# facebookresearch/habitat-lab

Hardware: NVIDIA H100
Metric: DD-PPO learner frames/sec (ResNet18 RGB-D 256x256) (higher is better)
Workload: dtype bf16

## Files before the change

habitat-lab_b200/csrc/conv.cu:

```cuda
#include "common.cuh"
#include "wgmma.cuh"

namespace hb200 {
void count_launch(int n);
static int g_umma_layout = 1;

using namespace wg;

constexpr int kStages = 3;
constexpr int kTileM = 128;
constexpr int kMaxBN = 128;
constexpr int kChunkK = 64;
constexpr int kMaxChunks = 512;

template <int LAYOUT>
__device__ __forceinline__ uint32_t tile_off(int row, int k8, int rows_total) {
  if (LAYOUT == 0) return (uint32_t)(k8 * rows_total + row) << 4;
  return (uint32_t)((row >> 3) << 10) + (uint32_t)((row & 7) << 7) + (uint32_t)((k8 ^ (row & 7)) << 4);
}
template <int LAYOUT>
__device__ __forceinline__ uint64_t kmajor_desc(uint32_t base, int kk, int rows_total) {
  if (LAYOUT == 0)
    return make_smem_desc(base + (uint32_t)(kk * 2 * rows_total * 16), (uint32_t)rows_total * 16, 128, kNoSwizzle);
  return make_smem_desc(base + (uint32_t)(kk * 32), 16, 1024, kSwizzle128B);
}
template <int LAYOUT>
constexpr uint32_t kmajor_hi() { return LAYOUT == 0 ? 8 * 128 : 8 * 1024; }

struct ConvArgs {
  const __nv_bfloat16* src;
  const __nv_bfloat16* wimg;
  __nv_bfloat16* out;
  const __nv_bfloat16* addend;
  double* stats;
  int B, SH, SW, SC;
  int OH, OW, OC;
  int kh, kw, stride, pad;
  int M, nchunks, cshift, gn_groups;
  const float* bias;
  int relu;
  int s2_classes;
  int wbn;
};

template <int BN, int MODE, int LAYOUT, int NST = kStages>
__global__ void __launch_bounds__(128) conv_igemm_kernel(const ConvArgs a) {
  extern __shared__ __align__(16) uint8_t smem_raw[];
  __shared__ float stage_buf[kStageFloats];
  constexpr uint32_t kABytes = kTileM * kChunkK * 2;
  constexpr uint32_t kBBytes = BN * kChunkK * 2;
  constexpr uint32_t kStageBytes = kABytes + kBBytes;
  static_assert(BN <= kMaxBN, "conv: N tile");
  const uint32_t smem_base = (smem_u32(smem_raw) + 1023u) & ~1023u;

  const int tid = threadIdx.x, lane = tid & 31;
  const int n0 = blockIdx.y * BN;
  __shared__ short chunk_ids[kMaxChunks];
  __shared__ int n_valid_s;
  int m, ob, op, oq, ph = 0, pw = 0;
  bool row_ok;
  if (MODE == 1 && a.s2_classes) {
    const int mq = a.M >> 2;
    const int tiles_per_class = (mq + kTileM - 1) / kTileM;
    const int cls = blockIdx.x / tiles_per_class;
    const int idx = (blockIdx.x - cls * tiles_per_class) * kTileM + tid;
    ph = cls >> 1; pw = cls & 1;
    row_ok = idx < mq;
    const int h2 = a.OH >> 1, w2 = a.OW >> 1;
    const int ii = row_ok ? idx : 0;
    ob = ii / (h2 * w2);
    const int rem = ii - ob * (h2 * w2);
    op = 2 * (rem / w2) + ph;
    oq = 2 * (rem % w2) + pw;
    m = (ob * a.OH + op) * a.OW + oq;
  } else {
    m = blockIdx.x * kTileM + tid;
    row_ok = m < a.M;
    const int hw = a.OH * a.OW;
    const int mm = row_ok ? m : 0;
    ob = mm / hw;
    const int rem = mm - ob * hw;
    op = rem / a.OW;
    oq = rem - op * a.OW;
  }
  __shared__ int4 row_info[kTileM];
  if (LAYOUT == 1) row_info[tid] = make_int4(ob, op, oq, row_ok ? 1 : 0);
  if (tid == 0) {
    int nv = 0;
    const int cpt = a.SC >> 6;
    for (int c = 0; c < a.nchunks && nv < kMaxChunks; ++c) {
      bool ok = true;
      if (MODE == 1 && a.s2_classes) {
        const int tap = c / cpt;
        const int r = tap / a.kw, sx = tap - r * a.kw;
        ok = tap < a.kh * a.kw && (((ph + a.pad - r) & 1) == 0) && (((pw + a.pad - sx) & 1) == 0);
      }
      if (ok) chunk_ids[nv++] = (short)c;
    }
    n_valid_s = nv;
  }

  __syncthreads();
  const int n_valid = n_valid_s;
  const int taps = a.kh * a.kw;
  const int wbn = a.wbn;
  const __nv_bfloat16* wtile =
// ... 748 lines not shown
```

habitat-lab_b200/csrc/conv_halo.cu:

```cuda
#include <cuda.h>
#include <stdlib.h>

#include "common.cuh"
#include "wgmma.cuh"

namespace hb200 {
void count_launch(int n);
using namespace wg;

constexpr int TH = 16, TW = 8;

__device__ __forceinline__ float warp_reduce16(float (&v)[16], int lane) {
  float a[8], b[4], c[2];
  const bool b4 = lane & 16, b3 = lane & 8, b2 = lane & 4, b1 = lane & 2;
#pragma unroll
  for (int i = 0; i < 8; ++i) a[i] = (b4 ? v[i + 8] : v[i]) + __shfl_xor_sync(0xffffffffu, b4 ? v[i] : v[i + 8], 16);
#pragma unroll
  for (int i = 0; i < 4; ++i) b[i] = (b3 ? a[i + 4] : a[i]) + __shfl_xor_sync(0xffffffffu, b3 ? a[i] : a[i + 4], 8);
#pragma unroll
  for (int i = 0; i < 2; ++i) c[i] = (b2 ? b[i + 2] : b[i]) + __shfl_xor_sync(0xffffffffu, b2 ? b[i] : b[i + 2], 4);
  float d = (b1 ? c[1] : c[0]) + __shfl_xor_sync(0xffffffffu, b1 ? c[0] : c[1], 2);
  d += __shfl_xor_sync(0xffffffffu, d, 1);
  return d;
}
// ... 806 lines not shown
            const uint64_t db = make_smem_desc(s_w + (r * KW + s) * (C * N * 2) + 2 * kk * (N * 16), N * 16, 128, kNoSwizzle);
            mma128<N, kT>(acc_t, da, 8 * ATOM, db, accum);
            accum = 1;
          }
      wgmma_commit();
      wgmma_wait<0>();
      acc_fence(acc_t);
    }
    if (NB == 1 && tid == 0 && it + 1 < my_n) issue_halo(first + (it + 1) * stride, 0);
    {
      int b, oh0, ow0;
      tile_coords(first + it * stride, b, oh0, ow0);
      const size_t pix = ((size_t)b * a.H + oh0 + py) * a.W + ow0 + px;
#pragma unroll
      for (int col0 = 0; col0 < N; col0 += 32) {
        float acc[32];
        acc_row32(acc_t, col0, stage_buf, acc);
        if (MODE == 0 && a.stats != nullptr)
          halo_gn_stats_chunk(acc, lane, N / a.gn_groups, a.stats + (size_t)b * a.gn_groups * 2, col0);
        const size_t o = pix * N + col0;
        if (MODE == 1 && a.addend != nullptr) {
          const uint4* ad = reinterpret_cast<const uint4*>(a.addend + o);
#pragma unroll
          for (int v = 0; v < 4; ++v) {
            float f[8];
            unpack8(ad[v], f);
#pragma unroll
            for (int e = 0; e < 8; ++e) acc[v * 8 + e] += f[e];
          }
        }
        uint4* dst = reinterpret_cast<uint4*>(a.y + o);
#pragma unroll
        for (int v = 0; v < 4; ++v) {
          uint4 u;
          if (MODE == 0) {
            u.x = pack_f16x2(acc[v * 8 + 0], acc[v * 8 + 1]);
            u.y = pack_f16x2(acc[v * 8 + 2], acc[v * 8 + 3]);
            u.z = pack_f16x2(acc[v * 8 + 4], acc[v * 8 + 5]);
            u.w = pack_f16x2(acc[v * 8 + 6], acc[v * 8 + 7]);
          } else {
            u.x = pack_bf16x2(acc[v * 8 + 0], acc[v * 8 + 1]);
            u.y = pack_bf16x2(acc[v * 8 + 2], acc[v * 8 + 3]);
            u.z = pack_bf16x2(acc[v * 8 + 4], acc[v * 8 + 5]);
            u.w = pack_bf16x2(acc[v * 8 + 6], acc[v * 8 + 7]);
          }
          dst[v] = u;
        }
      }
    }
  }
}


template <int C, int N, int KH, int KW, int PAD, int MODE, int NS, bool SW = false>
__global__ void __launch_bounds__(160)
conv_halo_ws_kernel(const HaloArgs a, const __grid_constant__ CUtensorMap tmap) {
  using Cfg = HaloCfg<C, N, KH, KW, PAD>;
  constexpr int CJ = Cfg::CJ, HH = Cfg::HH, HWD = Cfg::HWD;
  constexpr uint32_t SLAB = (uint32_t)((HH * HWD * 16 + 127) / 128 * 128);
  constexpr uint32_t RB = C * 2, ATOM = 8 * RB, COPY = HH * ATOM;
  constexpr uint32_t STAGE = SW ? KW * COPY : CJ * SLAB;
  constexpr int kSw = RB == 128 ? kSwizzle128B : kSwizzle64B;
  static_assert(!SW || RB == 64 || RB == 128, "swizzled halo copies: 32 or 64 channels");
  extern __shared__ __align__(16) uint8_t smem_raw[];
  __shared__ __align__(8) uint64_t full_bar[NS], empty_bar[NS];
  __shared__ float stage_buf[kStageFloats];
  const uint32_t sbase = (smem_u32(smem_raw) + 1023u) & ~1023u;
  const uint32_t s_w = sbase;
  const uint32_t s_halo0 = s_w + Cfg::W_BYTES;
  const int tid = threadIdx.x, warp = tid >> 5, lane = tid & 31;
  if (tid == 0) {
#pragma unroll
    for (int i = 0; i < NS; ++i) { mbar_init(&full_bar[i], 1); mbar_init(&empty_bar[i], 1); }
    mbar_fence_init();
  }
  {
    const uint4* src = reinterpret_cast<const uint4*>(a.wimg);
    for (int v = tid; v < Cfg::W_BYTES / 16; v += blockDim.x) cp_async16(s_w + (uint32_t)v * 16, src + v, true);
  }
  cp_async_commit();
  cp_async_wait<0>();
  fence_proxy_async_smem();
  __syncthreads();
  const int tiles_x = a.W / TW, tiles_per_img = tiles_x * (a.H / TH);
  const int first = blockIdx.x, stride = gridDim.x;
  const int my_n = first < a.ntiles ? (a.ntiles - first + stride - 1) / stride : 0;
  const CUtensorMap* const tmap_p = &tmap;

  if (warp == 4) {
    if (lane == 0) {
      for (int it = 0; it < my_n; ++it) {
        const int st = it % NS;
        if (it >= NS) mbar_wait(&empty_bar[st], ((it / NS) - 1) & 1);
        const int tile = first + it * stride;
        const int b = tile / tiles_per_img, r = tile - b * tiles_per_img;
        const int oh0 = (r / tiles_x) * TH, ow0 = (r % tiles_x) * TW;
        if constexpr (SW) {
          mbar_expect_tx(&full_bar[st], STAGE);
#pragma unroll
          for (int kx = 0; kx < KW; ++kx)
            tma_load_4d(s_halo0 + (uint32_t)st * STAGE + (uint32_t)kx * COPY, tmap_p, &full_bar[st], 0, ow0 - PAD + kx,
                        oh0 - PAD, b);
        } else {
          mbar_expect_tx(&full_bar[st], (uint32_t)(CJ * HH * HWD * 16));
#pragma unroll
          for (int j = 0; j < CJ; ++j)
            tma_load_4d(s_halo0 + (uint32_t)st * STAGE + (uint32_t)j * SLAB, tmap_p, &full_bar[st], j * 8, ow0 - PAD,
                        oh0 - PAD, b);
        }
      }
    }
    __syncwarp();
  } else {
    constexpr int kT = MODE == 0 ? kF16 : kBF16;
    const int py = tid >> 3, px = tid & 7;
    float acc_t[N];
    for (int it = 0; it < my_n; ++it) {
      const int st = it % NS;
      const int tile = first + it * stride;
      const int b = tile / tiles_per_img, r = tile - b * tiles_per_img;
      const int oh0 = (r / tiles_x) * TH, ow0 = (r % tiles_x) * TW;
      mbar_wait(&full_bar[st], (it / NS) & 1);
      const uint32_t sh = s_halo0 + (uint32_t)st * STAGE;
      wgmma_fence();
      uint32_t accum = 0;
#pragma unroll
      for (int r = 0; r < KH; ++r)
#pragma unroll
        for (int s = 0; s < KW; ++s)
#pragma unroll
          for (int kk = 0; kk < C / 16; ++kk) {
            const uint64_t da = SW ? make_smem_desc(sh + s * COPY + r * ATOM + kk * 32, 16, ATOM, (Layout)kSw)
                                   : make_smem_desc(sh + 2 * kk * SLAB + r * (HWD * 16) + s * 16, SLAB, HWD * 16, kNoSwizzle);
            const uint64_t db = make_smem_desc(s_w + (r * KW + s) * (C * N * 2) + 2 * kk * (N * 16), N * 16, 128, kNoSwizzle);
            mma128<N, kT>(acc_t, da, SW ? 8 * ATOM : 8 * HWD * 16, db, accum);
            accum = 1;
          }
      wgmma_commit();
      wgmma_wait<0>();
      acc_fence(acc_t);
      if (tid == 0) mbar_arrive(&empty_bar[st]);
      const size_t pix = ((size_t)b * a.H + oh0 + py) * a.W + ow0 + px;
#pragma unroll
      for (int col0 = 0; col0 < N; col0 += 32) {
        float acc_[32];
        acc_row32(acc_t, col0, stage_buf, acc_);
        if (MODE == 0 && a.stats != nullptr)
          halo_gn_stats_chunk(acc_, lane, N / a.gn_groups, a.stats + (size_t)b * a.gn_groups * 2, col0);
        const size_t o = pix * N + col0;
        if (MODE == 1 && a.addend != nullptr) {
          const uint4* ad = reinterpret_cast<const uint4*>(a.addend + o);
#pragma unroll
          for (int v = 0; v < 4; ++v) {
            float f[8];
            unpack8(ad[v], f);
#pragma unroll
            for (int e2 = 0; e2 < 8; ++e2) acc_[v * 8 + e2] += f[e2];
          }
        }
        uint4* dst = reinterpret_cast<uint4*>(a.y + o);
#pragma unroll
        for (int v = 0; v < 4; ++v) {
          uint4 u;
          if (MODE == 0) {
            u.x = pack_f16x2(acc_[v * 8 + 0], acc_[v * 8 + 1]);
            u.y = pack_f16x2(acc_[v * 8 + 2], acc_[v * 8 + 3]);
            u.z = pack_f16x2(acc_[v * 8 + 4], acc_[v * 8 + 5]);
            u.w = pack_f16x2(acc_[v * 8 + 6], acc_[v * 8 + 7]);
          } else {
            u.x = pack_bf16x2(acc_[v * 8 + 0], acc_[v * 8 + 1]);
            u.y = pack_bf16x2(acc_[v * 8 + 2], acc_[v * 8 + 3]);
            u.z = pack_bf16x2(acc_[v * 8 + 4], acc_[v * 8 + 5]);
            u.w = pack_bf16x2(acc_[v * 8 + 6], acc_[v * 8 + 7]);
          }
          dst[v] = u;
        }
      }
    }
  }
}

typedef CUresult (*EncodeTiledFn)(CUtensorMap*, CUtensorMapDataType, cuuint32_t, void*, const cuuint64_t*,
                                  const cuuint64_t*, const cuuint32_t*, const cuuint32_t*, CUtensorMapInterleave,
                                  CUtensorMapSwizzle, CUtensorMapL2promotion, CUtensorMapFloatOOBfill);
static EncodeTiledFn halo_encode_fn() {
  static EncodeTiledFn fn = nullptr;
  if (fn) return fn;
  void* p = nullptr;
  cudaDriverEntryPointQueryResult q;
  if (cudaGetDriverEntryPoint("cuTensorMapEncodeTiled", &p, cudaEnableDefault, &q) != cudaSuccess ||
      q != cudaDriverEntryPointSuccess)
    return nullptr;
  fn = (EncodeTiledFn)p;
  return fn;
}

static int blocks_per_sm(const void* kern, size_t smem, int* cache) {
  if (*cache > 0) return *cache;
  cudaFuncAttributes fa;
// ... 34 lines not shown
  }
  CUtensorMap tmap;
  const cuuint64_t dims[4] = {(cuuint64_t)C, (cuuint64_t)a.W, (cuuint64_t)a.H, (cuuint64_t)a.B};
  const cuuint64_t strides[3] = {(cuuint64_t)C * 2, (cuuint64_t)a.W * C * 2, (cuuint64_t)a.H * a.W * C * 2};
  const cuuint32_t box[4] = {8u, (cuuint32_t)Cfg::HWD, (cuuint32_t)Cfg::HH, 1u};
  const cuuint32_t estr[4] = {1u, 1u, 1u, 1u};
  const CUresult r = enc(&tmap, CU_TENSOR_MAP_DATA_TYPE_BFLOAT16, 4, (void*)a.x, dims, strides, box, estr,
                         CU_TENSOR_MAP_INTERLEAVE_NONE, CU_TENSOR_MAP_SWIZZLE_NONE, CU_TENSOR_MAP_L2_PROMOTION_L2_128B,
                         CU_TENSOR_MAP_FLOAT_OOB_FILL_NONE);
  if (r != CUDA_SUCCESS) {
    set_last_error("conv_halo (TMA): cuTensorMapEncodeTiled failed (%d)", (int)r);
    return HB200_ERR_CUDA;
  }
  constexpr size_t slab = (size_t)((Cfg::HH * Cfg::HWD * 16 + 127) / 128 * 128);
  constexpr int nstage = (Cfg::W_BYTES + 2 * (int)(Cfg::CJ * slab) > 110 * 1024) ? 1 : 2;
  const size_t smem = Cfg::W_BYTES + nstage * Cfg::CJ * slab + 256;
  auto kern = conv_halo_tma_kernel<C, N, KH, KW, PAD, MODE>;
  static int cache = 0;
  if (cache == 0) HB_CUDA(cudaFuncSetAttribute(kern, cudaFuncAttributeMaxDynamicSharedMemorySize, (int)smem));
  const int per_sm = blocks_per_sm((const void*)kern, smem, &cache);
  int grid = kNumSMs * per_sm;
  if (grid > a.ntiles) grid = a.ntiles;
  kern<<<grid, 128, smem, st>>>(a, tmap);
  HB_LAUNCH_OK();
  count_launch(1);
  return HB200_OK;
}

template <int C, int N, int KH, int KW, int PAD, int MODE, int NS, bool SW = false>
static int launch_halo_ws(const HaloArgs& a, cudaStream_t st) {
  using Cfg = HaloCfg<C, N, KH, KW, PAD>;
  EncodeTiledFn enc = halo_encode_fn();
  if (!enc) {
    set_last_error("conv_halo (TMA): cuTensorMapEncodeTiled is not available from this driver");
    return HB200_ERR_UNSUPPORTED;
  }
  CUtensorMap tmap;
  const cuuint64_t dims[4] = {(cuuint64_t)C, (cuuint64_t)a.W, (cuuint64_t)a.H, (cuuint64_t)a.B};
  const cuuint64_t strides[3] = {(cuuint64_t)C * 2, (cuuint64_t)a.W * C * 2, (cuuint64_t)a.H * a.W * C * 2};
  const cuuint32_t box_slab[4] = {8u, (cuuint32_t)Cfg::HWD, (cuuint32_t)Cfg::HH, 1u};
  const cuuint32_t box_rows[4] = {(cuuint32_t)C, (cuuint32_t)TW, (cuuint32_t)Cfg::HH, 1u};
  const cuuint32_t* box = SW ? box_rows : box_slab;
  const cuuint32_t estr[4] = {1u, 1u, 1u, 1u};
  const CUresult r = enc(&tmap, CU_TENSOR_MAP_DATA_TYPE_BFLOAT16, 4, (void*)a.x, dims, strides, box, estr,
                         CU_TENSOR_MAP_INTERLEAVE_NONE,
                         !SW ? CU_TENSOR_MAP_SWIZZLE_NONE : (C == 64 ? CU_TENSOR_MAP_SWIZZLE_128B : CU_TENSOR_MAP_SWIZZLE_64B),
                         CU_TENSOR_MAP_L2_PROMOTION_L2_128B, CU_TENSOR_MAP_FLOAT_OOB_FILL_NONE);
  if (r != CUDA_SUCCESS) {
    set_last_error("conv_halo (TMA): cuTensorMapEncodeTiled failed (%d)", (int)r);
    return HB200_ERR_CUDA;
  }
  constexpr size_t slab = (size_t)((Cfg::HH * Cfg::HWD * 16 + 127) / 128 * 128);
  const size_t stage = SW ? (size_t)KW * Cfg::HH * 8 * C * 2 : Cfg::CJ * slab;
  const size_t smem = Cfg::W_BYTES + (size_t)NS * stage + 1024;
  auto kern = conv_halo_ws_kernel<C, N, KH, KW, PAD, MODE, NS, SW>;
  static int grid_cache = 0;
  if (grid_cache == 0) {
    HB_CUDA(cudaFuncSetAttribute(kern, cudaFuncAttributeMaxDynamicSharedMemorySize, (int)smem));
    cudaFuncAttributes fa;
    HB_CUDA(cudaFuncGetAttributes(&fa, (const void*)kern));
    const int regs = fa.numRegs > 0 ? fa.numRegs : 128;
    int per_sm = 65536 / (((regs + 7) / 8 * 8) * 160);
    const int by_smem = (int)((227 * 1024) / (smem + fa.sharedSizeBytes + 1024));
    if (by_smem < per_sm) per_sm = by_smem;
    if (per_sm < 1) per_sm = 1;
    grid_cache = kNumSMs * per_sm;
  }
  const int grid = grid_cache < a.ntiles ? grid_cache : a.ntiles;
  kern<<<grid, 160, smem, st>>>(a, tmap);
  HB_LAUNCH_OK();
  count_launch(1);
  return HB200_OK;
}

template <int C, int N, int MODE>
static int launch_halo_sw(const HaloArgs& a, cudaStream_t st) {
  using Cfg = HaloCfg<C, N, 3, 3, 1>;
  EncodeTiledFn enc = halo_encode_fn();
  if (!enc) {
    set_last_error("conv_halo (swizzled TMA): cuTensorMapEncodeTiled is not available from this driver");
    return HB200_ERR_UNSUPPORTED;
  }
  CUtensorMap tmap;
  const cuuint64_t dims[4] = {(cuuint64_t)C, (cuuint64_t)a.W, (cuuint64_t)a.H, (cuuint64_t)a.B};
  const cuuint64_t strides[3] = {(cuuint64_t)C * 2, (cuuint64_t)a.W * C * 2, (cuuint64_t)a.H * a.W * C * 2};
  const cuuint32_t box[4] = {(cuuint32_t)C, (cuuint32_t)TW, (cuuint32_t)Cfg::HH, 1u};
  const cuuint32_t estr[4] = {1u, 1u, 1u, 1u};
  const CUresult r = enc(&tmap, CU_TENSOR_MAP_DATA_TYPE_BFLOAT16, 4, (void*)a.x, dims, strides, box, estr,
                         CU_TENSOR_MAP_INTERLEAVE_NONE, C == 64 ? CU_TENSOR_MAP_SWIZZLE_128B : CU_TENSOR_MAP_SWIZZLE_64B,
                         CU_TENSOR_MAP_L2_PROMOTION_L2_128B, CU_TENSOR_MAP_FLOAT_OOB_FILL_NONE);
  if (r != CUDA_SUCCESS) {
    set_last_error("conv_halo (swizzled TMA): cuTensorMapEncodeTiled failed (%d)", (int)r);
    return HB200_ERR_CUDA;
  }
  constexpr size_t stage = (size_t)3 * Cfg::HH * 8 * C * 2;
  constexpr int nstage = (Cfg::W_BYTES + 2 * (int)stage > 200 * 1024) ? 1 : 2;
  const size_t smem = Cfg::W_BYTES + nstage * stage + 1024;
  auto kern = conv_halo_sw_kernel<C, N, MODE>;
  static int cache = 0;
  if (cache == 0) HB_CUDA(cudaFuncSetAttribute(kern, cudaFuncAttributeMaxDynamicSharedMemorySize, (int)smem));
  const int per_sm = blocks_per_sm((const void*)kern, smem, &cache);
  int grid = kNumSMs * per_sm;
  if (grid > a.ntiles) grid = a.ntiles;
  kern<<<grid, 128, smem, st>>>(a, tmap);
  HB_LAUNCH_OK();
  count_launch(1);
  return HB200_OK;
}

template <int C, int N, int KH, int KW, int PAD, int XMODE = 0>
static int launch_halo_wgrad(const HaloWgradArgs& a, cudaStream_t st) {
  constexpr int CJ = C / 8, HWD = TW + KW - 1, P = HWD * 16, RP = CJ * P;
  constexpr int MT = (KH * CJ + 15) / 16, RMAX = (MT * 16 + CJ - 1) / CJ, HROWS = TH - 1 + RMAX;
  constexpr int STAGE = (128 * N * 2 + HROWS * RP + 1023) / 1024 * 1024;
  constexpr int NSW = halo_wgrad_stages(XMODE, C, STAGE);
  const size_t smem = NSW * (size_t)STAGE + 1024 + 64;
  EncodeTiledFn enc = halo_encode_fn();
  if (!enc) {
    set_last_error("conv_halo_wgrad: cuTensorMapEncodeTiled is not available from this driver");
    return HB200_ERR_UNSUPPORTED;
  }
  CUtensorMap tmap;
// ... 104 lines not shown
  g_halo_tma = enable;
  return HB200_OK;
}
extern "C" int hb200_get_halo_tma(void) { return g_halo_tma; }

extern "C" int hb200_conv_halo_supported(int c, int n, int k, int h, int w) {
  if (h % TH || w % TW) return 0;
  if (k == 3) return (c == 32 && n == 32) || (c == 64 && n == 64);
  if (k == 4) return c == 16 && n == 32;
  return 0;
}

extern "C" int hb200_conv_halo_wgrad_supported(int c, int n, int k, int h, int w) {
  if (hb200_conv_halo_supported(c, n, k, h, w)) return 1;
  return k == 3 && c % 32 == 0 && n % 128 == 0 && h == w && (h == 8 || h == 4);
}

extern "C" int hb200_pack_halo_weight(const float* w_oihw, hb200_bf16* img, int co, int ci_real, int c, int n,
                                      int k, int mode, hb200_stream_t stream) {
  HB_CHECK_ARG(w_oihw && img && mode >= 0 && mode <= 2, "pack_halo_weight: bad args");
  const long long total = (long long)k * k * c * n;
  pack_halo_weight_kernel<<<(int)min((total + 255) / 256, (long long)kNumSMs * 4), 256, 0, (cudaStream_t)stream>>>(
      w_oihw, (__nv_bfloat16*)img, k, k, c, n, co, ci_real, mode);
  HB_LAUNCH_OK();
  count_launch(1);
  return HB200_OK;
}

extern "C" int hb200_unpack_stem_wgrad(const float* dw_acc, float* dw_oihw, int co, int ci_real,
                                       hb200_stream_t stream) {
  HB_CHECK_ARG(dw_acc && dw_oihw && ci_real <= 4, "unpack_stem_wgrad: bad args");
  unpack_stem_wgrad_kernel<<<cdiv(co * ci_real * 49, 256), 256, 0, (cudaStream_t)stream>>>(dw_acc, dw_oihw, co, ci_real);
  HB_LAUNCH_OK();
  count_launch(1);
  return HB200_OK;
}

extern "C" int hb200_conv_halo(const hb200_bf16* x, const hb200_bf16* wimg, hb200_bf16* y, const hb200_bf16* addend,
                               double* gn_stats, int gn_groups, int batch, int h, int w, int c, int n, int k,
                               int mode, hb200_stream_t stream) {
  HB_CHECK_ARG(x && wimg && y, "conv_halo: null pointer");
  HB_CHECK_ARG(hb200_conv_halo_supported(c, n, k, h, w), "conv_halo: unsupported shape C=%d N=%d k=%d %dx%d", c, n, k, h, w);
  if (gn_stats) HB_CHECK_ARG(gn_groups > 0 && n % gn_groups == 0 && n / gn_groups >= 2, "conv_halo: bad GroupNorm groups");
  HaloArgs a;
  a.x = (const __nv_bfloat16*)x; a.wimg = (const __nv_bfloat16*)wimg; a.y = (__nv_bfloat16*)y;
  a.addend = (const __nv_bfloat16*)addend; a.stats = gn_stats;
  a.B = batch; a.H = h; a.W = w; a.gn_groups = gn_groups > 0 ? gn_groups : 1;
  a.ntiles = batch * (h / TH) * (w / TW);
  cudaStream_t st = (cudaStream_t)stream;
  const bool use_tma = g_halo_tma != 0;
  if (g_halo_tma == 1 && k == 3 && c == 64)
    return mode == 0 ? launch_halo_ws<64, 64, 3, 3, 1, 0, 2, true>(a, st) : launch_halo_ws<64, 64, 3, 3, 1, 1, 2, true>(a, st);
  if (g_halo_tma == 1 && k == 3 && c == 32)
    return mode == 0 ? launch_halo_ws<32, 32, 3, 3, 1, 0, 3, true>(a, st) : launch_halo_ws<32, 32, 3, 3, 1, 1, 3, true>(a, st);
  if (g_halo_tma == 1 && k == 4 && mode == 0) return launch_halo_ws<16, 32, 4, 4, 2, 0, 6>(a, st);
  if (g_halo_tma == 6 && k == 3 && c == 32)
    return mode == 0 ? launch_halo_ws<32, 32, 3, 3, 1, 0, 2, true>(a, st) : launch_halo_ws<32, 32, 3, 3, 1, 1, 2, true>(a, st);
  if (g_halo_tma == 4 && k == 3 && c == 32)
    return mode == 0 ? launch_halo_ws<32, 32, 3, 3, 1, 0, 3, true>(a, st) : launch_halo_ws<32, 32, 3, 3, 1, 1, 3, true>(a, st);
  if (g_halo_tma == 4 && k == 3 && c == 64)
    return mode == 0 ? launch_halo_ws<64, 64, 3, 3, 1, 0, 2, true>(a, st) : launch_halo_ws<64, 64, 3, 3, 1, 1, 2, true>(a, st);
  if (g_halo_tma == 3 && k == 3 && c == 32)
    return mode == 0 ? launch_halo_ws<32, 32, 3, 3, 1, 0, 4>(a, st) : launch_halo_ws<32, 32, 3, 3, 1, 1, 4>(a, st);
  if (g_halo_tma == 3 && k == 3 && c == 64)
    return mode == 0 ? launch_halo_ws<64, 64, 3, 3, 1, 0, 5>(a, st) : launch_halo_ws<64, 64, 3, 3, 1, 1, 5>(a, st);
  if (g_halo_tma == 3 && k == 4 && mode == 0) return launch_halo_ws<16, 32, 4, 4, 2, 0, 6>(a, st);
  if (g_halo_tma == 2 && k == 3 && c == 32)
    return mode == 0 ? launch_halo_sw<32, 32, 0>(a, st) : launch_halo_sw<32, 32, 1>(a, st);
  if (g_halo_tma == 2 && k == 3 && c == 64)
    return mode == 0 ? launch_halo_sw<64, 64, 0>(a, st) : launch_halo_sw<64, 64, 1>(a, st);
  if (use_tma && k == 3 && c == 32)
    return mode == 0 ? launch_halo_tma<32, 32, 3, 3, 1, 0>(a, st) : launch_halo_tma<32, 32, 3, 3, 1, 1>(a, st);
  if (use_tma && k == 4 && mode == 0) return launch_halo_tma<16, 32, 4, 4, 2, 0>(a, st);
  if (use_tma && k == 3 && c == 64)
    return mode == 0 ? launch_halo_tma<64, 64, 3, 3, 1, 0>(a, st) : launch_halo_tma<64, 64, 3, 3, 1, 1>(a, st);
  if (k == 3 && c == 32) return mode == 0 ? launch_halo<32, 32, 3, 3, 1, 0>(a, st) : launch_halo<32, 32, 3, 3, 1, 1>(a, st);
  if (k == 3 && c == 64) return mode == 0 ? launch_halo<64, 64, 3, 3, 1, 0>(a, st) : launch_halo<64, 64, 3, 3, 1, 1>(a, st);
  HB_CHECK_ARG(mode == 0, "conv_halo: the stem has no data gradient");
  return launch_halo<16, 32, 4, 4, 2, 0>(a, st);
}

__global__ void unpack_s2_wgrad_kernel(const float* __restrict__ acc, float* __restrict__ dw, int co, int ci) {
  const int total = co * ci * 9;
  for (int i = blockIdx.x * blockDim.x + threadIdx.x; i < total; i += gridDim.x * blockDim.x) {
    const int s = i % 3, r = (i / 3) % 3, c = (i / 9) % ci, o = i / (9 * ci);
    const int ky = r == 0 ? 0 : 1, dy = r == 0 ? 1 : r - 1, kx = s == 0 ? 0 : 1, dx = s == 0 ? 1 : s - 1;
    dw[i] = acc[((size_t)((ky * 2 + kx) * 4 + dy * 2 + dx) * ci + c) * co + o];
  }
}

extern "C" int hb200_conv_s2_wgrad_supported(int c, int n, int h, int w) {
  return c == 32 && n == 64 && h % (2 * TH) == 0 && w % (2 * TW) == 0;
}
extern "C" int hb200_conv_s2_wgrad(const hb200_bf16* x, const hb200_bf16* dy, float* dw_acc, int batch, int h, int w,
                                   int c, int n, hb200_stream_t stream) {
  HB_CHECK_ARG(x && dy && dw_acc && batch > 0, "conv_s2_wgrad: null pointer");
  HB_CHECK_ARG(hb200_conv_s2_wgrad_supported(c, n, h, w), "conv_s2_wgrad: unsupported shape C=%d N=%d %dx%d", c, n, h, w);
  HaloWgradArgs a;
  a.x = (const __nv_bfloat16*)x; a.dy = (const __nv_bfloat16*)dy; a.dw = dw_acc;
  a.B = batch; a.H = h / 2; a.W = w / 2;
  a.ntiles = batch * (a.H / TH) * (a.W / TW);
  return launch_halo_wgrad<128, 64, 2, 2, 1, 2>(a, (cudaStream_t)stream);
}
extern "C" int hb200_unpack_s2_wgrad(const float* dw_acc, float* dw_oihw, int co, int ci, hb200_stream_t stream) {
  HB_CHECK_ARG(dw_acc && dw_oihw && co > 0 && ci > 0, "unpack_s2_wgrad: bad args");
  unpack_s2_wgrad_kernel<<<cdiv(co * ci * 9, 256), 256, 0, (cudaStream_t)stream>>>(dw_acc, dw_oihw, co, ci);
  HB_LAUNCH_OK();
// ... 33 lines not shown
```

habitat-lab_b200/csrc/wgmma.cuh:

```cuda
#pragma once
#include <cuda_runtime.h>
#include <stdint.h>

namespace hb200 {
namespace wg {

__device__ __forceinline__ uint32_t smem_u32(const void* p) {
  return (uint32_t)__cvta_generic_to_shared(p);
}

enum Layout : uint32_t { kNoSwizzle = 0, kSwizzle128B = 2, kSwizzle64B = 4 };

__device__ __forceinline__ uint64_t make_smem_desc(uint32_t smem_addr, uint32_t lbo_bytes,
                                                   uint32_t sbo_bytes, uint32_t layout) {
  uint64_t d = 0;
  d |= (uint64_t)((smem_addr >> 4) & 0x3FFF);
  d |= (uint64_t)((lbo_bytes >> 4) & 0x3FFF) << 16;
  d |= (uint64_t)((sbo_bytes >> 4) & 0x3FFF) << 32;
  d |= (uint64_t)(layout & 7) << 61;
  return d;
}
__device__ __forceinline__ uint64_t desc_add(uint64_t d, uint32_t bytes) { return d + (uint64_t)(bytes >> 4); }

constexpr int kF16 = 0, kBF16 = 1, kTF32 = 2;
// ... 105 lines not shown
  template <int TA, int TB>
  static __device__ __forceinline__ void mma(float (&d)[64], uint64_t da, uint64_t db, uint32_t accum) {
    asm volatile(
        "{\n\t.reg .pred p;\n\tsetp.ne.b32 p, %66, 0;\n\t"
        "wgmma.mma_async.sync.aligned.m64n128k16.f32.f16.f16 "
        "{%0, %1, %2, %3, %4, %5, %6, %7, %8, %9, %10, %11, %12, %13, %14, %15, %16, %17, %18, %19, %20, %21, %22, %23, %24, %25, %26, %27, %28, %29, %30, %31, %32, %33, %34, %35, %36, %37, %38, %39, %40, %41, %42, %43, %44, %45, %46, %47, %48, %49, %50, %51, %52, %53, %54, %55, %56, %57, %58, %59, %60, %61, %62, %63}, %64, %65, p, 1, 1, %67, %68;\n\t}\n"
        : "+f"(d[0]), "+f"(d[1]), "+f"(d[2]), "+f"(d[3]), "+f"(d[4]), "+f"(d[5]), "+f"(d[6]), "+f"(d[7]), "+f"(d[8]), "+f"(d[9]), "+f"(d[10]), "+f"(d[11]), "+f"(d[12]), "+f"(d[13]), "+f"(d[14]), "+f"(d[15]), "+f"(d[16]), "+f"(d[17]), "+f"(d[18]), "+f"(d[19]), "+f"(d[20]), "+f"(d[21]), "+f"(d[22]), "+f"(d[23]), "+f"(d[24]), "+f"(d[25]), "+f"(d[26]), "+f"(d[27]), "+f"(d[28]), "+f"(d[29]), "+f"(d[30]), "+f"(d[31]), "+f"(d[32]), "+f"(d[33]), "+f"(d[34]), "+f"(d[35]), "+f"(d[36]), "+f"(d[37]), "+f"(d[38]), "+f"(d[39]), "+f"(d[40]), "+f"(d[41]), "+f"(d[42]), "+f"(d[43]), "+f"(d[44]), "+f"(d[45]), "+f"(d[46]), "+f"(d[47]), "+f"(d[48]), "+f"(d[49]), "+f"(d[50]), "+f"(d[51]), "+f"(d[52]), "+f"(d[53]), "+f"(d[54]), "+f"(d[55]), "+f"(d[56]), "+f"(d[57]), "+f"(d[58]), "+f"(d[59]), "+f"(d[60]), "+f"(d[61]), "+f"(d[62]), "+f"(d[63])
        : "l"(da), "l"(db), "r"(accum), "n"(TA), "n"(TB));
  }
};
template <> struct Wgmma<128, kF16 + 1> {
  template <int TA, int TB>
  static __device__ __forceinline__ void mma(float (&d)[64], uint64_t da, uint64_t db, uint32_t accum) {
    asm volatile(
        "{\n\t.reg .pred p;\n\tsetp.ne.b32 p, %66, 0;\n\t"
        "wgmma.mma_async.sync.aligned.m64n128k16.f32.bf16.bf16 "
        "{%0, %1, %2, %3, %4, %5, %6, %7, %8, %9, %10, %11, %12, %13, %14, %15, %16, %17, %18, %19, %20, %21, %22, %23, %24, %25, %26, %27, %28, %29, %30, %31, %32, %33, %34, %35, %36, %37, %38, %39, %40, %41, %42, %43, %44, %45, %46, %47, %48, %49, %50, %51, %52, %53, %54, %55, %56, %57, %58, %59, %60, %61, %62, %63}, %64, %65, p, 1, 1, %67, %68;\n\t}\n"
        : "+f"(d[0]), "+f"(d[1]), "+f"(d[2]), "+f"(d[3]), "+f"(d[4]), "+f"(d[5]), "+f"(d[6]), "+f"(d[7]), "+f"(d[8]), "+f"(d[9]), "+f"(d[10]), "+f"(d[11]), "+f"(d[12]), "+f"(d[13]), "+f"(d[14]), "+f"(d[15]), "+f"(d[16]), "+f"(d[17]), "+f"(d[18]), "+f"(d[19]), "+f"(d[20]), "+f"(d[21]), "+f"(d[22]), "+f"(d[23]), "+f"(d[24]), "+f"(d[25]), "+f"(d[26]), "+f"(d[27]), "+f"(d[28]), "+f"(d[29]), "+f"(d[30]), "+f"(d[31]), "+f"(d[32]), "+f"(d[33]), "+f"(d[34]), "+f"(d[35]), "+f"(d[36]), "+f"(d[37]), "+f"(d[38]), "+f"(d[39]), "+f"(d[40]), "+f"(d[41]), "+f"(d[42]), "+f"(d[43]), "+f"(d[44]), "+f"(d[45]), "+f"(d[46]), "+f"(d[47]), "+f"(d[48]), "+f"(d[49]), "+f"(d[50]), "+f"(d[51]), "+f"(d[52]), "+f"(d[53]), "+f"(d[54]), "+f"(d[55]), "+f"(d[56]), "+f"(d[57]), "+f"(d[58]), "+f"(d[59]), "+f"(d[60]), "+f"(d[61]), "+f"(d[62]), "+f"(d[63])
        : "l"(da), "l"(db), "r"(accum), "n"(TA), "n"(TB));
  }
};
template <> struct Wgmma<128, kTF32> {
  template <int TA, int TB>
  static __device__ __forceinline__ void mma(float (&d)[64], uint64_t da, uint64_t db, uint32_t accum) {
    static_assert(TA == 0 && TB == 0, "tf32 operands are K-major only");
    asm volatile(
        "{\n\t.reg .pred p;\n\tsetp.ne.b32 p, %66, 0;\n\t"
        "wgmma.mma_async.sync.aligned.m64n128k8.f32.tf32.tf32 "
        "{%0, %1, %2, %3, %4, %5, %6, %7, %8, %9, %10, %11, %12, %13, %14, %15, %16, %17, %18, %19, %20, %21, %22, %23, %24, %25, %26, %27, %28, %29, %30, %31, %32, %33, %34, %35, %36, %37, %38, %39, %40, %41, %42, %43, %44, %45, %46, %47, %48, %49, %50, %51, %52, %53, %54, %55, %56, %57, %58, %59, %60, %61, %62, %63}, %64, %65, p, 1, 1;\n\t}\n"
        : "+f"(d[0]), "+f"(d[1]), "+f"(d[2]), "+f"(d[3]), "+f"(d[4]), "+f"(d[5]), "+f"(d[6]), "+f"(d[7]), "+f"(d[8]), "+f"(d[9]), "+f"(d[10]), "+f"(d[11]), "+f"(d[12]), "+f"(d[13]), "+f"(d[14]), "+f"(d[15]), "+f"(d[16]), "+f"(d[17]), "+f"(d[18]), "+f"(d[19]), "+f"(d[20]), "+f"(d[21]), "+f"(d[22]), "+f"(d[23]), "+f"(d[24]), "+f"(d[25]), "+f"(d[26]), "+f"(d[27]), "+f"(d[28]), "+f"(d[29]), "+f"(d[30]), "+f"(d[31]), "+f"(d[32]), "+f"(d[33]), "+f"(d[34]), "+f"(d[35]), "+f"(d[36]), "+f"(d[37]), "+f"(d[38]), "+f"(d[39]), "+f"(d[40]), "+f"(d[41]), "+f"(d[42]), "+f"(d[43]), "+f"(d[44]), "+f"(d[45]), "+f"(d[46]), "+f"(d[47]), "+f"(d[48]), "+f"(d[49]), "+f"(d[50]), "+f"(d[51]), "+f"(d[52]), "+f"(d[53]), "+f"(d[54]), "+f"(d[55]), "+f"(d[56]), "+f"(d[57]), "+f"(d[58]), "+f"(d[59]), "+f"(d[60]), "+f"(d[61]), "+f"(d[62]), "+f"(d[63])
        : "l"(da), "l"(db), "r"(accum));
  }
};

__device__ __forceinline__ void wgmma_fence() { asm volatile("wgmma.fence.sync.aligned;" ::: "memory"); }
__device__ __forceinline__ void wgmma_commit() { asm volatile("wgmma.commit_group.sync.aligned;" ::: "memory"); }
template <int N>
__device__ __forceinline__ void wgmma_wait() {
  asm volatile("wgmma.wait_group.sync.aligned %0;" ::"n"(N) : "memory");
}
template <int N>
__device__ __forceinline__ void acc_fence(float (&acc)[N]) {
#pragma unroll
  for (int i = 0; i < N; ++i) asm volatile("" : "+f"(acc[i])::"memory");
}

template <int N, int T, int TA = 0, int TB = 0>
__device__ __forceinline__ void mma128(float (&acc)[N], uint64_t da, uint32_t a_hi, uint64_t db, uint32_t accum) {
  static_assert(N == 16 || N == 32 || N == 64 || N == 128, "wgmma tile width");
  Wgmma<N, T>::template mma<TA, TB>(*reinterpret_cast<float(*)[N / 2]>(&acc[0]), da, db, accum);
  Wgmma<N, T>::template mma<TA, TB>(*reinterpret_cast<float(*)[N / 2]>(&acc[N / 2]), desc_add(da, a_hi), db, accum);
}

__device__ __forceinline__ void wg_bar_sync() { asm volatile("bar.sync 1, 128;" ::: "memory"); }

constexpr int kStagePitch = 33;
constexpr int kStageFloats = 128 * kStagePitch;
template <int N>
__device__ __forceinline__ void acc_row32(const float (&acc)[N], int col0, float* stage, float (&r)[32]) {
  const int t = threadIdx.x & 127, w = t >> 5, l = t & 31;
  wg_bar_sync();
#pragma unroll
  for (int h = 0; h < 2; ++h) {
#pragma unroll
    for (int i = 0; i < 4; ++i) {
      const int idx = h * (N / 2) + ((col0 >> 3) + i) * 4;
      const int row = h * 64 + 16 * w + (l >> 2), col = 8 * i + 2 * (l & 3);
      stage[row * kStagePitch + col] = acc[idx];
      stage[row * kStagePitch + col + 1] = acc[idx + 1];
      stage[(row + 8) * kStagePitch + col] = acc[idx + 2];
      stage[(row + 8) * kStagePitch + col + 1] = acc[idx + 3];
    }
  }
  wg_bar_sync();
#pragma unroll
  for (int j = 0; j < 32; ++j) r[j] = stage[t * kStagePitch + j];
}

__device__ __forceinline__ void fence_proxy_async_smem() {
  asm volatile("fence.proxy.async.shared::cta;" ::: "memory");
}

__device__ __forceinline__ void mbar_init(uint64_t* bar, uint32_t count) {
  asm volatile("mbarrier.init.shared::cta.b64 [%0], %1;" ::"r"(smem_u32(bar)), "r"(count) : "memory");
}
__device__ __forceinline__ void mbar_fence_init() {
  asm volatile("fence.mbarrier_init.release.cluster;" ::: "memory");
}
__device__ __forceinline__ void mbar_arrive(uint64_t* bar) {
  asm volatile("mbarrier.arrive.shared::cta.b64 _, [%0];" ::"r"(smem_u32(bar)) : "memory");
}
__device__ __forceinline__ bool mbar_try_wait(uint64_t* bar, uint32_t parity) {
  uint32_t ok;
  asm volatile(
      "{\n\t"
      ".reg .pred p;\n\t"
      "mbarrier.try_wait.parity.shared::cta.b64 p, [%1], %2;\n\t"
      "selp.u32 %0, 1, 0, p;\n\t"
      "}\n"
      : "=r"(ok)
      : "r"(smem_u32(bar)), "r"(parity)
      : "memory");
  return ok != 0;
}
__device__ __forceinline__ void mbar_wait(uint64_t* bar, uint32_t parity) {
  if (mbar_try_wait(bar, parity)) return;
  const long long t0 = clock64();
  while (!mbar_try_wait(bar, parity)) {
    if (clock64() - t0 > 4000000000ll) __trap();
  }
}

__device__ __forceinline__ void mbar_expect_tx(uint64_t* bar, uint32_t bytes) {
  asm volatile("mbarrier.arrive.expect_tx.shared::cta.b64 _, [%0], %1;" ::"r"(smem_u32(bar)), "r"(bytes) : "memory");
}
__device__ __forceinline__ void tma_load_4d(uint32_t smem_dst, const void* tmap, uint64_t* bar, int c0, int c1,
                                            int c2, int c3) {
  asm volatile(
      "cp.async.bulk.tensor.4d.shared::cluster.global.tile.mbarrier::complete_tx::bytes [%0], [%1, {%3, %4, %5, %6}], [%2];"
      ::"r"(smem_dst), "l"(reinterpret_cast<uint64_t>(tmap)), "r"(smem_u32(bar)), "r"(c0), "r"(c1), "r"(c2), "r"(c3)
      : "memory");
}

__device__ __forceinline__ void tma_load_5d(uint32_t smem_dst, const void* tmap, uint64_t* bar, int c0, int c1, int c2,
                                            int c3, int c4) {
  asm volatile(
      "cp.async.bulk.tensor.5d.shared::cluster.global.tile.mbarrier::complete_tx::bytes [%0], [%1, {%3, %4, %5, %6, %7}], [%2];"
// ... 30 lines not shown
```

Before: 52090.

## Run two consumer warpgroups in halo conv kernel and move epilogue buffers to dynamic smem

The warp-specialized halo conv kernel grows from one consumer warpgroup to two, plus the producer warp (288 threads). The two consumers take alternating tiles, each with its own epilogue transpose buffer and named barrier, and the 32-channel path deepens the pipeline to 6 stages. The static stage buffer moves into dynamic shared memory: in the igemm kernel it aliases the pipeline stages, in the halo kernel it sits after the halo stages. The aim is to overlap one warpgroup's epilogue with the other's MMA, at the cost of more registers and shared memory per block, which may lower occupancy.

```diff
diff --git a/habitat-lab_b200/csrc/conv.cu b/habitat-lab_b200/csrc/conv.cu
--- a/habitat-lab_b200/csrc/conv.cu
+++ b/habitat-lab_b200/csrc/conv.cu
@@ -46,12 +46,13 @@
 template <int BN, int MODE, int LAYOUT, int NST = kStages>
 __global__ void __launch_bounds__(128) conv_igemm_kernel(const ConvArgs a) {
   extern __shared__ __align__(16) uint8_t smem_raw[];
-  __shared__ float stage_buf[kStageFloats];
   constexpr uint32_t kABytes = kTileM * kChunkK * 2;
   constexpr uint32_t kBBytes = BN * kChunkK * 2;
   constexpr uint32_t kStageBytes = kABytes + kBBytes;
   static_assert(BN <= kMaxBN, "conv: N tile");
+  static_assert(NST * kStageBytes >= kStageFloats * sizeof(float), "conv: epilogue transpose buffer");
   const uint32_t smem_base = (smem_u32(smem_raw) + 1023u) & ~1023u;
+  float* const stage_buf = reinterpret_cast<float*>(smem_raw + (smem_base - smem_u32(smem_raw)));
 
   const int tid = threadIdx.x, lane = tid & 31;
   const int n0 = blockIdx.y * BN;
diff --git a/habitat-lab_b200/csrc/conv_halo.cu b/habitat-lab_b200/csrc/conv_halo.cu
--- a/habitat-lab_b200/csrc/conv_halo.cu
+++ b/habitat-lab_b200/csrc/conv_halo.cu
@@ -882,8 +882,9 @@
 }
 
 
+constexpr int kHaloWsThreads = 288;
 template <int C, int N, int KH, int KW, int PAD, int MODE, int NS, bool SW = false>
-__global__ void __launch_bounds__(160)
+__global__ void __launch_bounds__(kHaloWsThreads)
 conv_halo_ws_kernel(const HaloArgs a, const __grid_constant__ CUtensorMap tmap) {
   using Cfg = HaloCfg<C, N, KH, KW, PAD>;
   constexpr int CJ = Cfg::CJ, HH = Cfg::HH, HWD = Cfg::HWD;
@@ -894,11 +895,11 @@
   static_assert(!SW || RB == 64 || RB == 128, "swizzled halo copies: 32 or 64 channels");
   extern __shared__ __align__(16) uint8_t smem_raw[];
   __shared__ __align__(8) uint64_t full_bar[NS], empty_bar[NS];
-  __shared__ float stage_buf[kStageFloats];
   const uint32_t sbase = (smem_u32(smem_raw) + 1023u) & ~1023u;
   const uint32_t s_w = sbase;
   const uint32_t s_halo0 = s_w + Cfg::W_BYTES;
   const int tid = threadIdx.x, warp = tid >> 5, lane = tid & 31;
+  float* const stage_bufs = reinterpret_cast<float*>(smem_raw + (s_halo0 + NS * STAGE - smem_u32(smem_raw)));
   if (tid == 0) {
 #pragma unroll
     for (int i = 0; i < NS; ++i) { mbar_init(&full_bar[i], 1); mbar_init(&empty_bar[i], 1); }
@@ -917,7 +918,7 @@
   const int my_n = first < a.ntiles ? (a.ntiles - first + stride - 1) / stride : 0;
   const CUtensorMap* const tmap_p = &tmap;
 
-  if (warp == 4) {
+  if (warp == 8) {
     if (lane == 0) {
       for (int it = 0; it < my_n; ++it) {
         const int st = it % NS;
@@ -943,9 +944,11 @@
     __syncwarp();
   } else {
     constexpr int kT = MODE == 0 ? kF16 : kBF16;
-    const int py = tid >> 3, px = tid & 7;
+    const int wgi = warp >> 2, t = tid & 127;
+    const int py = t >> 3, px = t & 7;
+    float* const stage_buf = stage_bufs + wgi * kStageFloats;
     float acc_t[N];
-    for (int it = 0; it < my_n; ++it) {
+    for (int it = wgi; it < my_n; it += 2) {
       const int st = it % NS;
       const int tile = first + it * stride;
       const int b = tile / tiles_per_img, r = tile - b * tiles_per_img;
@@ -969,12 +972,12 @@
       wgmma_commit();
       wgmma_wait<0>();
       acc_fence(acc_t);
-      if (tid == 0) mbar_arrive(&empty_bar[st]);
+      if (t == 0) mbar_arrive(&empty_bar[st]);
       const size_t pix = ((size_t)b * a.H + oh0 + py) * a.W + ow0 + px;
 #pragma unroll
       for (int col0 = 0; col0 < N; col0 += 32) {
         float acc_[32];
-        acc_row32(acc_t, col0, stage_buf, acc_);
+        acc_row32(acc_t, col0, stage_buf, acc_, 1 + wgi);
         if (MODE == 0 && a.stats != nullptr)
           halo_gn_stats_chunk(acc_, lane, N / a.gn_groups, a.stats + (size_t)b * a.gn_groups * 2, col0);
         const size_t o = pix * N + col0;
@@ -1115,7 +1118,7 @@
   }
   constexpr size_t slab = (size_t)((Cfg::HH * Cfg::HWD * 16 + 127) / 128 * 128);
   const size_t stage = SW ? (size_t)KW * Cfg::HH * 8 * C * 2 : Cfg::CJ * slab;
-  const size_t smem = Cfg::W_BYTES + (size_t)NS * stage + 1024;
+  const size_t smem = Cfg::W_BYTES + (size_t)NS * stage + 2 * kStageFloats * sizeof(float) + 1024;
   auto kern = conv_halo_ws_kernel<C, N, KH, KW, PAD, MODE, NS, SW>;
   static int grid_cache = 0;
   if (grid_cache == 0) {
@@ -1123,14 +1126,14 @@
     cudaFuncAttributes fa;
     HB_CUDA(cudaFuncGetAttributes(&fa, (const void*)kern));
     const int regs = fa.numRegs > 0 ? fa.numRegs : 128;
-    int per_sm = 65536 / (((regs + 7) / 8 * 8) * 160);
+    int per_sm = 65536 / (((regs + 7) / 8 * 8) * kHaloWsThreads);
     const int by_smem = (int)((227 * 1024) / (smem + fa.sharedSizeBytes + 1024));
     if (by_smem < per_sm) per_sm = by_smem;
     if (per_sm < 1) per_sm = 1;
     grid_cache = kNumSMs * per_sm;
   }
   const int grid = grid_cache < a.ntiles ? grid_cache : a.ntiles;
-  kern<<<grid, 160, smem, st>>>(a, tmap);
+  kern<<<grid, kHaloWsThreads, smem, st>>>(a, tmap);
   HB_LAUNCH_OK();
   count_launch(1);
   return HB200_OK;
@@ -1341,7 +1344,7 @@
   if (g_halo_tma == 1 && k == 3 && c == 64)
     return mode == 0 ? launch_halo_ws<64, 64, 3, 3, 1, 0, 2, true>(a, st) : launch_halo_ws<64, 64, 3, 3, 1, 1, 2, true>(a, st);
   if (g_halo_tma == 1 && k == 3 && c == 32)
-    return mode == 0 ? launch_halo_ws<32, 32, 3, 3, 1, 0, 3, true>(a, st) : launch_halo_ws<32, 32, 3, 3, 1, 1, 3, true>(a, st);
+    return mode == 0 ? launch_halo_ws<32, 32, 3, 3, 1, 0, 6, true>(a, st) : launch_halo_ws<32, 32, 3, 3, 1, 1, 6, true>(a, st);
   if (g_halo_tma == 1 && k == 4 && mode == 0) return launch_halo_ws<16, 32, 4, 4, 2, 0, 6>(a, st);
   if (g_halo_tma == 6 && k == 3 && c == 32)
     return mode == 0 ? launch_halo_ws<32, 32, 3, 3, 1, 0, 2, true>(a, st) : launch_halo_ws<32, 32, 3, 3, 1, 1, 2, true>(a, st);
diff --git a/habitat-lab_b200/csrc/wgmma.cuh b/habitat-lab_b200/csrc/wgmma.cuh
--- a/habitat-lab_b200/csrc/wgmma.cuh
+++ b/habitat-lab_b200/csrc/wgmma.cuh
@@ -181,14 +181,14 @@
   Wgmma<N, T>::template mma<TA, TB>(*reinterpret_cast<float(*)[N / 2]>(&acc[N / 2]), desc_add(da, a_hi), db, accum);
 }
 
-__device__ __forceinline__ void wg_bar_sync() { asm volatile("bar.sync 1, 128;" ::: "memory"); }
+__device__ __forceinline__ void wg_bar_sync(int id) { asm volatile("bar.sync %0, 128;" ::"r"(id) : "memory"); }
 
 constexpr int kStagePitch = 33;
 constexpr int kStageFloats = 128 * kStagePitch;
 template <int N>
-__device__ __forceinline__ void acc_row32(const float (&acc)[N], int col0, float* stage, float (&r)[32]) {
+__device__ __forceinline__ void acc_row32(const float (&acc)[N], int col0, float* stage, float (&r)[32], int bar = 1) {
   const int t = threadIdx.x & 127, w = t >> 5, l = t & 31;
-  wg_bar_sync();
+  wg_bar_sync(bar);
 #pragma unroll
   for (int h = 0; h < 2; ++h) {
 #pragma unroll
@@ -201,7 +201,7 @@
       stage[(row + 8) * kStagePitch + col + 1] = acc[idx + 3];
     }
   }
-  wg_bar_sync();
+  wg_bar_sync(bar);
 #pragma unroll
   for (int j = 0; j < 32; ++j) r[j] = stage[t * kStagePitch + j];
 }
```

Result: faster. 54820 (median of 6 runs) (+5.2%).
